# huggingface/parler-tts

Hardware: NVIDIA H100
Metric: audio codec tokens/sec (all codebooks) (higher is better)
Workload: dtype bf16

## Files before the change

### parler_tts_b200/csrc/step2.cu

```cuda
#include "attn_core.cuh"
#include "common.cuh"
#include "kernels.h"
#include "ln_stats.cuh"
#include "sample_core.cuh"
#include "ptx.cuh"
#include "step.h"
#include "step_common.cuh"
#include <type_traits>

namespace ptts {
namespace cl {

constexpr int C = 2;
constexpr int V = 8;
constexpr int THREADS = 256;
constexpr int ROWS = 32;
constexpr int HROWS = 8;
constexpr int ATT_SMEM = attn_decode_smem_per_warp<bf16>();
constexpr int PROF_STRIDE = 16;
constexpr int QMAX = 6;
constexpr int OFF_STATS = 256, OFF_PART = 512, OFF_RES = 2560, OFF_CVEC = 3584;
constexpr int HDR = 5632;
constexpr int WB_BYTES = 65536;
constexpr int R_OFF = HDR + 2 * WB_BYTES;
constexpr int R_BYTES = 92160;
constexpr int R_PASS0 = 65536;
constexpr int QKV_OFF = R_BYTES - 2048;
constexpr int SMEM_BYTES = R_OFF + R_BYTES;
static_assert(SMEM_BYTES + 1024 <= 227 * 1024, "cluster step kernel shared memory");
static_assert(ROWS * (1024 / 2 + 8) * 2 <= V * (256 + ROWS * 34 * 4) && 2 * V * (256 + ROWS * 34 * 4) <= R_BYTES, "fc1 plan");
static_assert(2 * V * C * (32 + 4 * 96 * 4) <= R_PASS0 && R_PASS0 + V * QMAX * 32 * 16 <= QKV_OFF, "QKV plan");
static_assert(5 * ATT_SMEM <= QKV_OFF && 3 * ATT_SMEM <= WB_BYTES && 16384 + 4 * 128 * 4 <= WB_BYTES, "attention plan");
static_assert(ROWS * (4096 / 4 + 8) * 2 + V * (256 + ROWS * 8 * 4) <= R_BYTES, "fc2 plan");

__device__ __forceinline__ void mbar_wait(uint64_t* bar, uint32_t parity, int what) {
  uint32_t ok, spins = 0;
  do {
    ok = mbar_try_wait_cluster(bar, parity);
    if (!ok && ++spins > (1u << 22)) { printf("ptts: cluster step mbarrier timeout (cta %d, barrier kind %d)\n", (int)blockIdx.x, what); __trap(); }
  } while (!ok);
}
__device__ __forceinline__ void bulk_s2peer(uint32_t dst_cluster_addr, const void* src_smem, uint32_t bytes, uint32_t bar_cluster_addr) {
  asm volatile("cp.async.bulk.shared::cluster.shared::cta.mbarrier::complete_tx::bytes [%0], [%1], %2, [%3];"
               ::"r"(dst_cluster_addr), "r"(smem_u32(src_smem)), "r"(bytes), "r"(bar_cluster_addr) : "memory");
}
__device__ __forceinline__ uint32_t mapa(uint32_t addr, uint32_t rank) { uint32_t r; asm volatile("mapa.shared::cluster.u32 %0, %1, %2;" : "=r"(r) : "r"(addr), "r"(rank)); return r; }
__device__ __forceinline__ uint32_t cluster_rank() { uint32_t r; asm volatile("mov.u32 %0, %%cluster_ctarank;" : "=r"(r)); return r; }
__device__ __forceinline__ void cluster_arrive() { asm volatile("barrier.cluster.arrive.release.aligned;" ::: "memory"); }
__device__ __forceinline__ void cluster_wait() { asm volatile("barrier.cluster.wait.acquire.aligned;" ::: "memory"); }
__device__ __forceinline__ void cluster_arrive_reuse() { asm volatile("barrier.cluster.arrive.relaxed.aligned;" ::: "memory"); }

__host__ __device__ __forceinline__ int kslice(int kt) { return (kt & 7) >> 2; }
__host__ __device__ __forceinline__ int klocal(int kt) { return ((kt >> 3) << 2) | (kt & 3); }
__host__ __device__ __forceinline__ int kglobal(int rank, int lk) { return ((lk >> 2) << 3) | (rank << 2) | (lk & 3); }

template <int QN, int MT, bool STATS, bool ACC = false>
__device__ __forceinline__ void mma_slice(float (&out)[2][6][4], RowStatFrag& rst, const bf16* xs, int apitch, const uint4* wb, int KT, int kt0,
                                          int kt_end, int lrow, int lcol) {
  float acc[MT][QN][4];
#pragma unroll
  for (int a = 0; a < MT; a++)
#pragma unroll
    for (int j = 0; j < QN; j++)
#pragma unroll
      for (int e = 0; e < 4; e++) acc[a][j][e] = ACC ? out[a][j][e] : 0.f;
  for (int kt = kt0; kt < kt_end; kt += 4) {
    uint32_t a[MT][2][4];
#pragma unroll
    for (int mt = 0; mt < MT; mt++)
#pragma unroll
      for (int j = 0; j < 2; j++) ldmatrix_x4(a[mt][j], xs + (size_t)(mt * 16 + lrow) * apitch + kt * 32 + j * 16 + lcol);
    if (STATS) {
#pragma unroll
      for (int mt = 0; mt < MT; mt++) { row_stat_mma(rst, mt, a[mt][0]); row_stat_mma(rst, mt, a[mt][1]); }
    }
#pragma unroll
    for (int j = 0; j < QN; j++) {
      const uint4 w = wb[((size_t)j * KT + kt) * 32];
#pragma unroll
      for (int mt = 0; mt < MT; mt++) {
        mma_bf16_16816(acc[mt][j], a[mt][0], w.x, w.y);
        mma_bf16_16816(acc[mt][j], a[mt][1], w.z, w.w);
      }
    }
  }
#pragma unroll
  for (int mt = 0; mt < MT; mt++)
#pragma unroll
    for (int j = 0; j < QN; j++)
#pragma unroll
      for (int e = 0; e < 4; e++) out[mt][j][e] = acc[mt][j][e];
}

enum { PH_QKV = 0, PH_O = 1, PH_QC = 2, PH_OC = 3, PH_FC1 = 4, PH_FC2 = 5 };
constexpr int JOBS_PER_LAYER = 9;
constexpr int QKV_JOBS = 4;

__device__ __forceinline__ bool weight_job(const StepParams& p, int j, int cta, int rank, const char*& src, uint32_t& bytes) {
  const int nl = JOBS_PER_LAYER * p.L;
  if (j < nl) {
    const int l = j / JOBS_PER_LAYER, jl = j - JOBS_PER_LAYER * l;
    const int ph = jl < QKV_JOBS ? 0 : jl - (QKV_JOBS - 1);
    const int64_t idx = (ph == PH_QKV || ph == PH_QC) ? (int64_t)(cta >> 3) * C + rank : (int64_t)cta;
    const int64_t sz = p.cp_slice[ph];
    bytes = (uint32_t)(ph == PH_QKV ? sz / QKV_JOBS : sz);
    src = p.blob + p.layer0 + p.layer_stride * l + p.cp[ph] + idx * sz + (ph == PH_QKV ? jl * (sz / QKV_JOBS) : 0);
    return true;
  }
  const int task = cta + (int)gridDim.x * (j - nl);
  const int ntasks = p.K * p.V / 32;
  if (task >= ntasks) return false;
  bytes = (uint32_t)(4 * p.H * 16);
  src = p.blob + p.heads + (int64_t)task * bytes;
  return true;
}

template <int ITEMS>
__global__ void __launch_bounds__(THREADS, 1) decode_step_cluster_kernel(const __grid_constant__ StepParams p) {
  extern __shared__ __align__(128) unsigned char smem[];
  Ctrl* ctrl = p.sa.ctrl;
  if (p.prof != nullptr && blockIdx.x == 0 && threadIdx.x == 0) p.prof[(size_t)(6 * p.L + 2) * PROF_STRIDE + 3] = clock64();
  if (ctrl->active == 0) return;
  int cur_len = ctrl->cur_len;
  const unsigned gen = (unsigned)ctrl->launch_gen;
  int pos = p.P + cur_len - 1;
  const int tid = threadIdx.x, warp = tid >> 5, lane = tid & 31;
  const int H = p.H, F = p.F, B = p.B;
  const int rank = (int)cluster_rank();
  const int cta = (int)blockIdx.x;
  const int cluster = cta >> 1;
  const int head = cluster >> 2, rblk = cluster & 3;
  const int Ks = H / C, KsF = F / 4;
  const int pitch = Ks + 8, pitchF = KsF + 8;
  const int qe = F / p.nh / 64;
  const int dgrp = warp & 1, e4 = warp >> 1;

  uint64_t* abar = reinterpret_cast<uint64_t*>(smem);
  uint64_t* wbar = abar + 1;
  uint64_t* xbar = abar + 3;
  uint64_t* attbars = reinterpret_cast<uint64_t*>(smem + 128);
  float* stats = reinterpret_cast<float*>(smem + OFF_STATS);
  float* part = reinterpret_cast<float*>(smem + OFF_PART);
  float* res_s = reinterpret_cast<float*>(smem + OFF_RES);
  float* cvec = reinterpret_cast<float*>(smem + OFF_CVEC);
  unsigned char* Rg = smem + R_OFF;
  uint32_t par_a = 0, par_w = 0, par_x = 0, att_parity = 0;

  if (tid == 0) {
    mbar_init<1>(abar); mbar_init<1>(&wbar[0]); mbar_init<1>(&wbar[1]); mbar_init<1>(xbar);
    asm volatile("fence.mbarrier_init.release.cluster;" ::: "memory");
  }
  attention_decode_init_warp(attbars + 2 * warp, lane);
  cluster_arrive(); cluster_wait();
  unsigned* const bar_ctr = p.bar + (gen & 1u);
  unsigned bar_target = 0u;
  if (cta == 0 && tid == 0) p.bar[(gen + 1u) & 1u] = 0u;

  const char* blob = p.blob;
  long long* const prof0 = (p.prof != nullptr && cta == 0) ? p.prof : nullptr;
  long long* prof = prof0;
  prof_mark(prof, 0);

  auto issue_weight_job = [&](int j) {
    const char* src; uint32_t bytes;
    if (!weight_job(p, j, cta, rank, src, bytes)) return;
    mbar_expect_tx(&wbar[j & 1], bytes);
    bulk_g2s_evict_first(smem + HDR + (j & 1) * WB_BYTES, src, bytes, &wbar[j & 1]);
  };
  __shared__ int s_next_active;
  const int n_steps = (p.do_sample_phase && p.n_steps > 1 && prof0 == nullptr) ? p.n_steps : 1;
  int unfinished_prev = 0;
#pragma unroll 1
  for (int it = 0; it < n_steps; it++) {
  pos = p.P + cur_len - 1;
  prof = prof0;
  cluster_arrive_reuse();
  if (tid == 0) { issue_weight_job(0); issue_weight_job(1); }

  bf16* const x_img = p.cl_x;
  bf16* const a_img = p.cl_attn;
  bf16* const h_img = p.cl_h;
  const int x_slice_elems = ROWS * pitch, h_slice_elems = ROWS * pitchF;
  auto h_offset = [&](int n) {
    const int lk = klocal(n >> 5), kq = KsF >> 5;
    return (size_t)(2 * kslice(n >> 5) + lk / kq) * h_slice_elems + (lk % kq) * 32 + (n & 31);
  };
  const int xo_slice = kslice(cta >> 2), xo_col = klocal(cta >> 2) * 32 + (cta & 3) * 8;

  {
    const int row = tid >> 3, f = tid & 7, n = cta * 8 + f;
    const float v = row < B ? embed_value(p, row, n, pos) : 0.f;
    res_s[row * 8 + f] = v;
    x_img[(size_t)xo_slice * x_slice_elems + row * pitch + xo_col + f] = __float2bfloat16_rn(v);
  }
  prof_mark(prof, 6);
  auto request_slice = [&](const bf16* img_slice, uint32_t bytes) {
    fence_proxy_async_smem();
    mbar_expect_tx(abar, bytes);
    bulk_g2s(Rg, img_slice, bytes, abar);
  };
  auto slice_of = [&](int sub, const bf16*& img, uint32_t& bytes) {
    if (sub == PH_QKV || sub == PH_QC) { img = x_img + (size_t)rank * x_slice_elems + (size_t)(HROWS * rblk) * pitch; bytes = (uint32_t)(HROWS * pitch * 2); }
    else if (sub == PH_O || sub == PH_OC) { img = a_img + (size_t)rank * x_slice_elems; bytes = (uint32_t)(x_slice_elems * 2); }
    else if (sub == PH_FC1) { img = x_img + (size_t)rank * x_slice_elems; bytes = (uint32_t)(x_slice_elems * 2); }
    else { img = h_img + (size_t)(2 * rank) * h_slice_elems; bytes = (uint32_t)(h_slice_elems * 2); }
  };
  {
    const bf16* nimg; uint32_t nbytes;
    slice_of(PH_QKV, nimg, nbytes);
    bar_target = grid_sync(bar_ctr, bar_target, -1, false, nullptr, [&]() { request_slice(nimg, nbytes); });
  }
  prof_mark(prof, 7);

  const int lrow = (lane & 7) + ((lane >> 3) & 1) * 8, lcol = (lane >> 4) * 8;
  const int g = lane >> 2, t4 = lane & 3;
  const int n_phases = 6 * p.L;

  const int att_row = HROWS * rblk + 4 * rank + (warp >> 1);
  const int att_slice = kslice(2 * head), att_col = klocal(2 * head) * 32;

#pragma unroll 1
  for (int ph = 0; ph < n_phases; ph++) {
    const int l = ph / 6, sub = ph - 6 * l;
    prof = prof0 ? prof0 + (size_t)(ph + 1) * PROF_STRIDE : nullptr;
    prof_mark(prof, 0);
    const char* lb = blob + p.layer0 + p.layer_stride * l;
    const bool rowpart = (sub == PH_QKV || sub == PH_QC);
    const bool has_ln = (sub == PH_QKV || sub == PH_QC || sub == PH_FC1);
    const int q = (sub == PH_QKV) ? 6 : (sub == PH_QC ? 2 : (sub == PH_FC1 ? qe : 1));
    const int Nc = 4 * q * 8;
    const int KT = (sub == PH_FC2 ? KsF : Ks) >> 5;
    const int apitch = (sub == PH_FC2) ? pitchF : pitch;
    const int act_bytes = (rowpart ? HROWS : ROWS) * apitch * 2;
    const int RS = (q == 1) ? 8 : 8 * q + 2;
    const int blk = rowpart ? 32 + 4 * 16 * q * 4 : 256 + ROWS * RS * 4;
    const int wsend = rowpart ? C * blk : blk;
    const int j0 = JOBS_PER_LAYER * l + (sub == 0 ? 0 : sub + QKV_JOBS - 1);

    float cv1 = 0.f, cv2 = 0.f;
    if (has_ln) {
      const float* c1; int ntot;
      if (sub == PH_QKV) { c1 = reinterpret_cast<const float*>(lb + p.c_qkv); ntot = p.qkv_rows; }
      else if (sub == PH_QC) { c1 = reinterpret_cast<const float*>(lb + p.c_qc); ntot = H; }
      else { c1 = reinterpret_cast<const float*>(lb + p.c_fc1); ntot = F; }
      const int nown = rowpart ? Nc : 8 * q;
      if (tid < nown) {
        int n;
        if (sub == PH_QKV) n = (tid >> 6) * (p.nh * HD) + head * HD + (tid & 63);
        else if (sub == PH_QC) n = head * HD + tid;
        else n = cta * 8 * q + tid;
        cv1 = c1[n];
        cv2 = c1[ntot + n];
      }
    }

    auto wait_job = [&](int j) {
      mbar_wait(&wbar[j & 1], (par_w >> (j & 1)) & 1u, 1);
      par_w ^= 1u << (j & 1);
    };
    auto ring = [&](int j) { return reinterpret_cast<const uint4*>(smem + HDR + (j & 1) * WB_BYTES) + lane; };
    wait_job(j0);
    if (sub == PH_QKV) wait_job(j0 + 1);
    mbar_wait(abar, par_a, 0);
    par_a ^= 1u;
    prof_mark(prof, 1);
    float acc[2][QMAX][4];
    float4* const pass0 = reinterpret_cast<float4*>(Rg + R_PASS0) + (size_t)warp * QMAX * 32 + lane;
    RowStatFrag rst;
    row_stat_zero(rst);
    {
      const bf16* xs = reinterpret_cast<const bf16*>(Rg);
      if (rowpart) {
        auto head_pass = [&](auto pass_tag) {
          constexpr int P = decltype(pass_tag)::value;
          const int u = 2 * P + dgrp;
          float t[2][QMAX][4];
          if (sub == PH_QKV) mma_slice<6, 1, P == 0>(t, rst, xs, apitch, ring(j0 + u), KT, e4, KT, lrow & 7, lcol);
          else mma_slice<2, 1, P == 0>(t, rst, xs, apitch, ring(j0) + (size_t)(2 * u) * KT * 32, KT, e4, KT, lrow & 7, lcol);
#pragma unroll
          for (int j = 0; j < QMAX; j++)
            if (j < q) {
              if (P == 0) pass0[j * 32] = make_float4(t[0][j][0], t[0][j][1], t[0][j][2], t[0][j][3]);
              else {
#pragma unroll
                for (int e = 0; e < 4; e++) acc[0][j][e] = t[0][j][e];
              }
            }
        };
        head_pass(std::integral_constant<int, 0>{});
        if (sub == PH_QKV) {
          prof_mark(prof, 8);
          __syncthreads();
          if (tid == 0) { issue_weight_job(j0 + 2); issue_weight_job(j0 + 3); }
          wait_job(j0 + 2);
          wait_job(j0 + 3);
          prof_mark(prof, 9);
        }
        head_pass(std::integral_constant<int, 1>{});
      } else if (sub == PH_FC2) {
        auto quarter = [&](auto qq_tag) {
          constexpr int QQ = decltype(qq_tag)::value;
          const uint4* wq = ring(j0) + (size_t)dgrp * 2 * KT * 32 + (size_t)QQ * KT * 32;
          mma_slice<1, 2, false, QQ == 1>(acc, rst, xs, apitch, wq, 2 * KT, (e4 - QQ * KT) & 3, KT, lrow, lcol);
        };
        quarter(std::integral_constant<int, 0>{});
        prof_mark(prof, 8);
        __syncthreads();
        if (tid == 0) request_slice(h_img + (size_t)(2 * rank + 1) * h_slice_elems, (uint32_t)(h_slice_elems * 2));
        mbar_wait(abar, par_a, 0);
        par_a ^= 1u;
        prof_mark(prof, 9);
        quarter(std::integral_constant<int, 1>{});
      } else {
        const uint4* wb = ring(j0) + (size_t)(dgrp * q) * KT * 32;
        if (sub == PH_FC1) {
          if (q == 4) mma_slice<4, 2, true>(acc, rst, xs, apitch, wb, KT, e4, KT, lrow, lcol);
          else if (q == 2) mma_slice<2, 2, true>(acc, rst, xs, apitch, wb, KT, e4, KT, lrow, lcol);
          else mma_slice<1, 2, true>(acc, rst, xs, apitch, wb, KT, e4, KT, lrow, lcol);
        } else mma_slice<1, 2, false>(acc, rst, xs, apitch, wb, KT, e4, KT, lrow, lcol);
      }
    }
    prof_mark(prof, 2);
    if (has_ln && tid < (rowpart ? Nc : 8 * q)) { cvec[tid] = cv1; cvec[256 + tid] = cv2; }
    __syncthreads();
    prof_mark(prof, 12);
    cluster_wait();
    prof_mark(prof, 13);

    const int nslots = rowpart ? V * C : V;
    unsigned char* send = Rg;
    const int send_end = V * wsend;
    unsigned char* recv = Rg + (((send_end > act_bytes ? send_end : act_bytes) + 127) & ~127);
    if (tid == 0) mbar_expect_tx(xbar, (uint32_t)(nslots * blk));
    {
      unsigned char* mine = send + (size_t)warp * wsend;
      if (!rowpart) {
        float* bp = reinterpret_cast<float*>(mine + 256);
#pragma unroll
        for (int mt = 0; mt < 2; mt++)
#pragma unroll
          for (int j = 0; j < QMAX; j++) {
            if (j < q) {
              float* base = bp + (size_t)(mt * 16 + g) * RS + j * 8 + 2 * t4;
              *reinterpret_cast<float2*>(base) = make_float2(acc[mt][j][0], acc[mt][j][1]);
              *reinterpret_cast<float2*>(base + 8 * RS) = make_float2(acc[mt][j][2], acc[mt][j][3]);
            }
          }
        if (has_ln) {
          float* st = reinterpret_cast<float*>(mine);
#pragma unroll
          for (int mt = 0; mt < 2; mt++) {
            const int r0 = mt * 16 + g;
            if (t4 == 0) { st[2 * r0] = rst.s1[mt][0]; st[2 * (r0 + 8)] = rst.s1[mt][2]; }
            if (t4 == (g >> 1)) {
              st[2 * r0 + 1] = (g & 1) ? rst.sq[mt][0][1] : rst.sq[mt][0][0];
              st[2 * (r0 + 8) + 1] = (g & 1) ? rst.sq[mt][1][3] : rst.sq[mt][1][2];
            }
          }
        }
      } else {
        const int qc = 16 * q;
        unsigned char* blk_d = send + ((size_t)(g >> 2) * V + warp) * blk;
        float* bp = reinterpret_cast<float*>(blk_d + 32) + (g & 3) * qc + 2 * t4;
#pragma unroll
        for (int P = 0; P < 2; P++)
#pragma unroll
          for (int j = 0; j < QMAX; j++)
            if (j < q) *reinterpret_cast<float2*>(bp + P * 8 * q + j * 8) = P == 0 ? make_float2(pass0[j * 32].x, pass0[j * 32].y)
                                                                                   : make_float2(acc[0][j][0], acc[0][j][1]);
        float* st = reinterpret_cast<float*>(blk_d) + (g & 3) * 2;
        if (t4 == 0) st[0] = rst.s1[0][0];
        if (t4 == (g >> 1)) st[1] = (g & 1) ? rst.sq[0][0][1] : rst.sq[0][0][0];
      }
      __syncwarp();
      prof_mark(prof, 14);
      if (!rowpart) {
        if (lane == 0) {
          fence_proxy_async_smem();
          bulk_s2peer(mapa(smem_u32(recv + (size_t)(4 * rank + e4) * blk), (uint32_t)dgrp), mine, (uint32_t)blk, mapa(smem_u32(xbar), (uint32_t)dgrp));
        }
      } else {
        __syncthreads();
        if (warp < C && lane == 0) {
          fence_proxy_async_smem();
          bulk_s2peer(mapa(smem_u32(recv + (size_t)(8 * rank) * blk), (uint32_t)warp), send + (size_t)warp * V * blk, (uint32_t)(V * blk), mapa(smem_u32(xbar), (uint32_t)warp));
        }
      }
    }
    if (warp == 1 && lane == 0 && !rowpart && sub != PH_OC) issue_weight_job(j0 + 2);
    if (warp == 1 && lane == 0 && sub == PH_QKV) issue_weight_job(j0 + QKV_JOBS);
    prof_mark(prof, 15);
    mbar_wait(xbar, par_x, 2);
    par_x ^= 1u;
    prof_mark(prof, 3);

    if (!rowpart) {
      const int row = tid >> 3, f0 = tid & 7;
      float ln_mean = 0.f, ln_rstd = 0.f;
      if (has_ln) {
        float S1 = 0.f, S2 = 0.f;
#pragma unroll
        for (int v = 0; v < V; v++) { const float2 x = *reinterpret_cast<const float2*>(recv + (size_t)v * blk + row * 8); S1 += x.x; S2 += x.y; }
        ln_mean = S1 / (float)H;
        ln_rstd = rsqrtf(fmaxf(S2 / (float)H - ln_mean * ln_mean, 0.f) + p.eps);
      }
      if (row < B && sub == PH_FC1 && q == 4) {
        const int f = 4 * f0;
        float v[4] = {0.f, 0.f, 0.f, 0.f};
#pragma unroll
        for (int sv = 0; sv < V; sv++) {
          const float* bp = reinterpret_cast<const float*>(recv + (size_t)sv * blk + 256) + row * RS + f;
          const float2 a = *reinterpret_cast<const float2*>(bp), b2 = *reinterpret_cast<const float2*>(bp + 2);
          v[0] += a.x; v[1] += a.y; v[2] += b2.x; v[3] += b2.y;
        }
#pragma unroll
        for (int e = 0; e < 4; e++) v[e] = apply_act(DT<bf16>::rnd(ln_rstd * (v[e] - ln_mean * cvec[f + e]) + cvec[256 + f + e]), p.act);
        uint2 pk;
        pk.x = att_pack(v[0], v[1]); pk.y = att_pack(v[2], v[3]);
        *reinterpret_cast<uint2*>(h_img + h_offset(cta * 32 + f) + row * pitchF) = pk;
      } else if (row < B) {
        for (int i = 0; i < q; i++) {
          const int f = f0 + 8 * i;
          float v = 0.f;
#pragma unroll
          for (int sv = 0; sv < V; sv++) v += reinterpret_cast<const float*>(recv + (size_t)sv * blk + 256)[row * RS + f];
          if (sub == PH_FC1) {
            v = ln_rstd * (v - ln_mean * cvec[f]) + cvec[256 + f];
            v = apply_act(DT<bf16>::rnd(v), p.act);
            h_img[h_offset(cta * 8 * q + f) + row * pitchF] = __float2bfloat16_rn(v);
          } else {
            v = DT<bf16>::rnd(res_s[row * 8 + f] + DT<bf16>::rnd(v));
            res_s[row * 8 + f] = v;
            x_img[(size_t)xo_slice * x_slice_elems + row * pitch + xo_col + f] = __float2bfloat16_rn(v);
          }
        }
      }
    } else {
      bf16* qkv_s = reinterpret_cast<bf16*>(Rg + QKV_OFF);
      auto gather = [&](auto jw_tag) {
        constexpr int JW = decltype(jw_tag)::value, NC = 4 * JW, QCW = 2 * JW;
        for (int idx = tid; idx < 4 * NC; idx += THREADS) {
          const int r4 = idx / NC, col = idx - r4 * NC;
          const int u = col / JW, cw = (u >> 1) * JW + (col - u * JW);
          float S1 = 0.f, S2 = 0.f;
#pragma unroll
          for (int e = 0; e < V; e++) {
            const float2 x = *reinterpret_cast<const float2*>(recv + (size_t)(8 * (e >> 2) + 2 * (e & 3)) * blk + r4 * 8);
            S1 += x.x; S2 += x.y;
          }
          const float ln_mean = S1 / (float)H;
          const float ln_rstd = rsqrtf(fmaxf(S2 / (float)H - ln_mean * ln_mean, 0.f) + p.eps);
          float v = 0.f;
#pragma unroll
          for (int e = 0; e < V; e++)
            v += reinterpret_cast<const float*>(recv + (size_t)(8 * (e >> 2) + 2 * (e & 3) + (u & 1)) * blk + 32)[r4 * QCW + cw];
          v = ln_rstd * (v - ln_mean * cvec[col]) + cvec[256 + col];
          qkv_s[idx] = __float2bfloat16_rn(v);
        }
      };
      if (sub == PH_QKV) gather(std::integral_constant<int, 48>{}); else gather(std::integral_constant<int, 16>{});
      static_assert(HD == 64, "QKV: 2 x 2 units of 6 n-tiles (q|k|v of a head), q_cross: 2 x 2 units of 2 n-tiles");
    }
    prof_mark(prof, 4);
    __syncthreads();
    cluster_arrive_reuse();
    if (rowpart) {
      cluster_wait();
      cluster_arrive();
    }

    if (rowpart) {
      if (att_row < B) {
        AttnArgs att = decode_attn_args(p, l, pos, sub == PH_QC);
        const bf16* qkv_s = reinterpret_cast<const bf16*>(Rg + QKV_OFF);
        const int row_base = HROWS * rblk + 4 * rank;
        const bf16* qbase = qkv_s - (size_t)row_base * Nc - (size_t)head * HD;
        att.q = qbase; att.ldq = Nc;
        att.ldo = pitch;
        att.out = a_img + (size_t)att_slice * x_slice_elems + att_col - (size_t)head * HD;
        if (sub == PH_QKV) { att.knew = qbase; att.vnew = qbase; att.ldkv = Nc; att.k_col0 = HD; att.v_col0 = 2 * HD; }
        unsigned char* wb0 = smem + HDR;
        unsigned char* held = wb0 + ((sub == PH_QKV ? j0 + 1 : j0) & 1) * WB_BYTES;
        unsigned char* other = wb0 + ((sub == PH_QKV ? j0 : j0 + 1) & 1) * WB_BYTES;
        unsigned char* region = warp < 5 ? Rg + (size_t)warp * ATT_SMEM : held + (size_t)(warp - 5) * ATT_SMEM;
        float* xr = reinterpret_cast<float*>(other + 16384) + (warp >> 1) * 128;
        attention_decode_item_warp<bf16>(att, att_row, head, pos, region, attbars + 2 * warp, lane, att_parity, warp & 1, 2, xr, (warp >> 1) + 1);
      }
      prof_mark(prof, 5);
    }
    prof_mark(prof, 6);
    if (p.prof != nullptr && l == p.L / 2 && tid == 0) {
      unsigned long long ns;
      asm volatile("mov.u64 %0, %%globaltimer;" : "=l"(ns));
      p.prof[(size_t)(n_phases + 4) * PROF_STRIDE + sub * (int)gridDim.x + cta] = (long long)ns;
    }

    const bool last = (ph + 1 == n_phases);
    const bf16* nimg; uint32_t nbytes;
    if (last) { nimg = x_img; nbytes = (uint32_t)(C * x_slice_elems * 2); }
    else slice_of((sub + 1) % 6, nimg, nbytes);
    const int held_job = sub == PH_QKV ? j0 + QKV_JOBS + 1 : (sub == PH_QC || sub == PH_OC) ? j0 + 2 : -1;
    bar_target = grid_sync(bar_ctr, bar_target, ph, false, nullptr, [&]() {
      request_slice(nimg, nbytes);
      if (held_job >= 0) issue_weight_job(held_job);
    });
    prof_mark(prof, 7);
  }
  cluster_wait();

  prof = prof0 ? prof0 + (size_t)(n_phases + 1) * PROF_STRIDE : nullptr;
  prof_mark(prof, 0);
  {
    const int ntasks = p.K * p.V / 32;
    const float* c1 = reinterpret_cast<const float*>(blob + p.c_heads);
    const float* c2 = c1 + p.K * p.V;
    mbar_wait(abar, par_a, 3);
    par_a ^= 1u;
    const bf16* xs = reinterpret_cast<const bf16*>(Rg);
    const int KTH = H >> 5;
    auto ktile = [&](int kt) { return xs + (size_t)kslice(kt) * x_slice_elems + klocal(kt) * 32; };
    {
      RowStatFrag rst;
      row_stat_zero(rst);
      for (int kt = warp; kt < KTH; kt += 8) {
        const bf16* sl = ktile(kt);
#pragma unroll
        for (int mt = 0; mt < 2; mt++)
#pragma unroll
          for (int j = 0; j < 2; j++) {
            uint32_t a[4];
            ldmatrix_x4(a, sl + (size_t)(mt * 16 + lrow) * pitch + j * 16 + lcol);
            row_stat_mma(rst, mt, a);
          }
      }
      row_stat_store(rst, part, warp, lane);
      __syncthreads();
      row_stat_finalize(part, H, ROWS, p.eps, stats);
      __syncthreads();
    }
    prof_mark(prof, 1);
    constexpr int HRS = 40;
    int job = JOBS_PER_LAYER * p.L;
    for (int task = cta; task < ntasks; task += (int)gridDim.x, job++) {
      mbar_wait(&wbar[job & 1], (par_w >> (job & 1)) & 1u, 4);
      par_w ^= 1u << (job & 1);
      float acc[2][4][4];
#pragma unroll
      for (int a = 0; a < 2; a++)
#pragma unroll
        for (int j = 0; j < 4; j++)
#pragma unroll
          for (int e = 0; e < 4; e++) acc[a][j][e] = 0.f;
      unsigned char* wbuf = smem + HDR + (job & 1) * WB_BYTES;
      const uint4* wb = reinterpret_cast<const uint4*>(wbuf) + lane;
      for (int kt = warp; kt < KTH; kt += 8) {
        const bf16* sl = ktile(kt);
        uint32_t a[2][2][4];
#pragma unroll
        for (int mt = 0; mt < 2; mt++)
#pragma unroll
          for (int j = 0; j < 2; j++) ldmatrix_x4(a[mt][j], sl + (size_t)(mt * 16 + lrow) * pitch + j * 16 + lcol);
#pragma unroll
        for (int j = 0; j < 4; j++) {
          const uint4 w = wb[((size_t)j * KTH + kt) * 32];
#pragma unroll
          for (int mt = 0; mt < 2; mt++) {
            mma_bf16_16816(acc[mt][j], a[mt][0], w.x, w.y);
            mma_bf16_16816(acc[mt][j], a[mt][1], w.z, w.w);
          }
        }
      }
      __syncthreads();
      float* red = reinterpret_cast<float*>(wbuf);
#pragma unroll
      for (int mt = 0; mt < 2; mt++)
#pragma unroll
        for (int j = 0; j < 4; j++) {
          float* base = red + ((size_t)warp * 32 + mt * 16 + g) * HRS + j * 8 + 2 * t4;
          *reinterpret_cast<float2*>(base) = make_float2(acc[mt][j][0], acc[mt][j][1]);
          *reinterpret_cast<float2*>(base + 8 * HRS) = make_float2(acc[mt][j][2], acc[mt][j][3]);
        }
      __syncthreads();
      {
        const int er = tid >> 3, ec = tid & 7;
        if (er < B) {
          const float mean = stats[2 * er], rstd = stats[2 * er + 1];
#pragma unroll
          for (int j = 0; j < 4; j++) {
            const int cidx = j * 8 + ec, n = task * 32 + cidx;
            float v = 0.f;
#pragma unroll
            for (int w = 0; w < 8; w++) v += red[((size_t)w * 32 + er) * HRS + cidx];
            p.logits[(size_t)er * p.K * p.V + n] = DT<bf16>::rnd(rstd * (v - mean * c1[n]) + c2[n]);
          }
        }
      }
      __syncthreads();
      if (tid == 32) {
        fence_proxy_async_smem();
        issue_weight_job(job + 2);
      }
    }
  }
  prof_mark(prof, 6);
  bar_target = grid_sync(bar_ctr, bar_target, n_phases, true);
  prof = prof0 ? prof0 + (size_t)(n_phases + 2) * PROF_STRIDE : nullptr;
  prof_mark(prof, 0);
  if (p.do_sample_phase) {
    const ptts_gen_params gp = *p.sa.gen;
    const int BK = B * p.K;
    sample_phase<ITEMS>(p.sa, gp, BK, cur_len);
    prof_mark(prof, 1);
    bar_target = grid_sync(bar_ctr, bar_target, n_phases + 1, true, nullptr, [&]() {
      const int tot = *reinterpret_cast<volatile int*>(&ctrl->n_unfinished);
      s_next_active = (tot - unfinished_prev > 0) ? 1 : 0;
      unfinished_prev = tot;
    });
    prof_mark(prof, 2);
  }
  bool go_on = false;
  if (p.do_sample_phase) {
    const int act = s_next_active;
    if (cta == 0 && tid == 0) {
      ctrl->cur_len = cur_len + 1;
      ctrl->active = act;
      ctrl->steps_run += 1;
    }
    go_on = act != 0;
    cur_len += 1;
  }
  if (!go_on) break;
  }
  if (cta == 0 && tid == 0) {
    if (p.do_sample_phase) ctrl->n_unfinished = 0;
    ctrl->launch_gen = (int)(gen + 1u);
  }
}

__global__ void cluster_pack_kernel(const uint4* __restrict__ src, uint4* __restrict__ dst, int ph, int nh, int ntc, int kts, int KT_src) {
  const int64_t tile = blockIdx.x;
  const int ktl = (int)(tile % kts);
  const int j = (int)((tile / kts) % ntc);
  const int slice = (int)(tile / ((int64_t)kts * ntc));
  const int rank = slice & 1, owner = slice >> 1;
  int n_tile;
  if (ph == PH_QKV) n_tile = (j >> 3) * (nh * 8) + owner * 8 + (j & 7);
  else n_tile = owner * ntc + j;
  const int kt = kglobal(rank, ktl);
  dst[tile * 32 + threadIdx.x] = src[((int64_t)n_tile * KT_src + kt) * 32 + threadIdx.x];
}

}

int cluster_pack_layer(const char* layer_src, char* layer_dst, const int64_t* mat_off, const int64_t* cp_off, int nh, int H, int F, cudaStream_t st) {
  const int ks = H / cl::C / 32, ksf = F / cl::C / 32;
  const int ntc[6] = {24, 2, 8, 2, F / (4 * nh) / 8, 2};
  const int owners[6] = {nh, 4 * nh, nh, 4 * nh, 4 * nh, 4 * nh};
  for (int ph = 0; ph < 6; ph++) {
    const int kts = (ph == 5) ? ksf : ks;
    const int KT_src = (ph == 5) ? F / 32 : H / 32;
    const int64_t tiles = (int64_t)owners[ph] * cl::C * ntc[ph] * kts;
    cl::cluster_pack_kernel<<<(unsigned)tiles, 32, 0, st>>>(reinterpret_cast<const uint4*>(layer_src + mat_off[ph]),
                                                            reinterpret_cast<uint4*>(layer_dst + cp_off[ph]), ph, nh, ntc[ph], kts, KT_src);
  }
  PTTS_LAUNCH_CHECK();
  return PTTS_OK;
}

static const void* cluster_kernel_fn(const StepParams& p) {
  if (p.sample_items <= 1) return (const void*)cl::decode_step_cluster_kernel<1>;
  if (p.sample_items <= 5) return (const void*)cl::decode_step_cluster_kernel<5>;
  return (const void*)cl::decode_step_cluster_kernel<9>;
}

static void cluster_launch_config(const StepParams& p, cudaLaunchConfig_t& cfg, cudaLaunchAttribute* at, cudaStream_t st) {
  cfg = cudaLaunchConfig_t{};
  cfg.gridDim = dim3((unsigned)(4 * p.nh * cl::C));
  cfg.blockDim = dim3(cl::THREADS);
  cfg.dynamicSmemBytes = cl::SMEM_BYTES;
  cfg.stream = st;
  at[0].id = cudaLaunchAttributeClusterDimension;
  at[0].val.clusterDim.x = cl::C; at[0].val.clusterDim.y = 1; at[0].val.clusterDim.z = 1;
  at[1].id = cudaLaunchAttributeCooperative;
  at[1].val.cooperative = 1;
  cfg.attrs = at;
  cfg.numAttrs = 2;
}

bool cluster_step_available(const StepParams& p) {
  const void* fn = cluster_kernel_fn(p);
  static bool told = false;
  auto why = [&](const char* what, cudaError_t e, int n) {
    if (!told) fprintf(stderr, "ptts_b200: cluster step kernel not used (%s: %s, %d co-resident clusters of %d, need %d); the one-CTA-per-SM step kernel runs instead\n",
                       what, cudaGetErrorString(e), n, cl::C, 4 * p.nh);
    told = true;
    cudaGetLastError();
    return false;
  };
  cudaError_t e = cudaFuncSetAttribute(fn, cudaFuncAttributeMaxDynamicSharedMemorySize, cl::SMEM_BYTES);
  if (e != cudaSuccess) return why("shared memory attribute", e, 0);
  cudaLaunchConfig_t cfg; cudaLaunchAttribute at[2];
  cluster_launch_config(p, cfg, at, nullptr);
  cfg.numAttrs = 1;
  int n = 0;
  e = cudaOccupancyMaxActiveClusters(&n, fn, &cfg);
  if (e != cudaSuccess) return why("cluster occupancy query", e, n);
  if (n < 4 * p.nh) return why("too few co-resident clusters", cudaSuccess, n);
  return true;
}

int launch_decode_step_cluster(const StepParams& p, cudaStream_t st) {
  const void* fn = cluster_kernel_fn(p);
  cudaLaunchConfig_t cfg; cudaLaunchAttribute at[2];
  cluster_launch_config(p, cfg, at, st);
  void* args[] = {(void*)&p};
  PTTS_CHECK_CUDA(cudaLaunchKernelExC(&cfg, fn, args));
  return PTTS_OK;
}

}
```

Baseline: 228,500.

## Exchange partial GEMM results via per-thread st.async into peer CTA shared memory

Replaces the staged exchange of partial matmul results and layernorm stats with direct st.async stores from registers into the peer CTA's receive buffer (or local stores for the own rank). Previously these were written to a local send buffer, then moved with a bulk cp.async after syncthreads and syncwarp. The change drops the send staging area, the pass-0 spill buffer, and an extra cluster wait/arrive round in row-partitioned phases. The mbarrier expected-tx count is now computed analytically, so it must match the number of bytes actually stored remotely. That adds many small remote stores and some ordering risk around cluster_wait placement.

```diff
diff --git a/parler_tts_b200/csrc/step2.cu b/parler_tts_b200/csrc/step2.cu
--- a/parler_tts_b200/csrc/step2.cu
+++ b/parler_tts_b200/csrc/step2.cu
@@ -24,12 +24,11 @@
 constexpr int WB_BYTES = 65536;
 constexpr int R_OFF = HDR + 2 * WB_BYTES;
 constexpr int R_BYTES = 92160;
-constexpr int R_PASS0 = 65536;
 constexpr int QKV_OFF = R_BYTES - 2048;
 constexpr int SMEM_BYTES = R_OFF + R_BYTES;
 static_assert(SMEM_BYTES + 1024 <= 227 * 1024, "cluster step kernel shared memory");
-static_assert(ROWS * (1024 / 2 + 8) * 2 <= V * (256 + ROWS * 34 * 4) && 2 * V * (256 + ROWS * 34 * 4) <= R_BYTES, "fc1 plan");
-static_assert(2 * V * C * (32 + 4 * 96 * 4) <= R_PASS0 && R_PASS0 + V * QMAX * 32 * 16 <= QKV_OFF, "QKV plan");
+static_assert(ROWS * (1024 / 2 + 8) * 2 + V * (256 + ROWS * 34 * 4) <= R_BYTES, "fc1 plan");
+static_assert(HROWS * (1024 / 2 + 8) * 2 + V * C * (32 + 4 * 96 * 4) <= QKV_OFF, "QKV plan");
 static_assert(5 * ATT_SMEM <= QKV_OFF && 3 * ATT_SMEM <= WB_BYTES && 16384 + 4 * 128 * 4 <= WB_BYTES, "attention plan");
 static_assert(ROWS * (4096 / 4 + 8) * 2 + V * (256 + ROWS * 8 * 4) <= R_BYTES, "fc2 plan");
 
@@ -40,9 +39,13 @@
     if (!ok && ++spins > (1u << 22)) { printf("ptts: cluster step mbarrier timeout (cta %d, barrier kind %d)\n", (int)blockIdx.x, what); __trap(); }
   } while (!ok);
 }
-__device__ __forceinline__ void bulk_s2peer(uint32_t dst_cluster_addr, const void* src_smem, uint32_t bytes, uint32_t bar_cluster_addr) {
-  asm volatile("cp.async.bulk.shared::cluster.shared::cta.mbarrier::complete_tx::bytes [%0], [%1], %2, [%3];"
-               ::"r"(dst_cluster_addr), "r"(smem_u32(src_smem)), "r"(bytes), "r"(bar_cluster_addr) : "memory");
+__device__ __forceinline__ void st_async(uint32_t dst_cluster_addr, float v, uint32_t bar_cluster_addr) {
+  asm volatile("st.async.shared::cluster.mbarrier::complete_tx::bytes.b32 [%0], %1, [%2];"
+               ::"r"(dst_cluster_addr), "r"(__float_as_uint(v)), "r"(bar_cluster_addr) : "memory");
+}
+__device__ __forceinline__ void st_async(uint32_t dst_cluster_addr, float2 v, uint32_t bar_cluster_addr) {
+  asm volatile("st.async.shared::cluster.mbarrier::complete_tx::bytes.v2.f32 [%0], {%1, %2}, [%3];"
+               ::"r"(dst_cluster_addr), "f"(v.x), "f"(v.y), "r"(bar_cluster_addr) : "memory");
 }
 __device__ __forceinline__ uint32_t mapa(uint32_t addr, uint32_t rank) { uint32_t r; asm volatile("mapa.shared::cluster.u32 %0, %1, %2;" : "=r"(r) : "r"(addr), "r"(rank)); return r; }
 __device__ __forceinline__ uint32_t cluster_rank() { uint32_t r; asm volatile("mov.u32 %0, %%cluster_ctarank;" : "=r"(r)); return r; }
@@ -126,7 +129,7 @@
   int pos = p.P + cur_len - 1;
   const int tid = threadIdx.x, warp = tid >> 5, lane = tid & 31;
   const int H = p.H, F = p.F, B = p.B;
-  const int rank = (int)cluster_rank();
+  const int rank = (int)cluster_rank(), peer = rank ^ 1;
   const int cta = (int)blockIdx.x;
   const int cluster = cta >> 1;
   const int head = cluster >> 2, rblk = cluster & 3;
@@ -144,6 +147,7 @@
   float* res_s = reinterpret_cast<float*>(smem + OFF_RES);
   float* cvec = reinterpret_cast<float*>(smem + OFF_CVEC);
   unsigned char* Rg = smem + R_OFF;
+  const uint32_t peer_xbar = mapa(smem_u32(xbar), (uint32_t)peer);
   uint32_t par_a = 0, par_w = 0, par_x = 0, att_parity = 0;
 
   if (tid == 0) {
@@ -234,8 +238,15 @@
     const int act_bytes = (rowpart ? HROWS : ROWS) * apitch * 2;
     const int RS = (q == 1) ? 8 : 8 * q + 2;
     const int blk = rowpart ? 32 + 4 * 16 * q * 4 : 256 + ROWS * RS * 4;
-    const int wsend = rowpart ? C * blk : blk;
+    unsigned char* const recv = Rg + ((act_bytes + 127) & ~127);
+    const uint32_t peer_recv = mapa(smem_u32(recv), (uint32_t)peer);
+    const uint32_t xbytes = 4u * (rowpart ? V * 4 * 16 * q + V / 2 * 4 * 2 : V / C * (ROWS * 8 * q + (has_ln ? ROWS * 2 : 0)));
+    auto put = [&](int d, uint32_t off, auto v) {
+      if (d == rank) *reinterpret_cast<decltype(v)*>(recv + off) = v;
+      else st_async(peer_recv + off, v, peer_xbar);
+    };
     const int j0 = JOBS_PER_LAYER * l + (sub == 0 ? 0 : sub + QKV_JOBS - 1);
+    if (tid == 0) mbar_expect_tx(xbar, xbytes);
 
     float cv1 = 0.f, cv2 = 0.f;
     if (has_ln) {
@@ -265,7 +276,6 @@
     par_a ^= 1u;
     prof_mark(prof, 1);
     float acc[2][QMAX][4];
-    float4* const pass0 = reinterpret_cast<float4*>(Rg + R_PASS0) + (size_t)warp * QMAX * 32 + lane;
     RowStatFrag rst;
     row_stat_zero(rst);
     {
@@ -277,15 +287,19 @@
           float t[2][QMAX][4];
           if (sub == PH_QKV) mma_slice<6, 1, P == 0>(t, rst, xs, apitch, ring(j0 + u), KT, e4, KT, lrow & 7, lcol);
           else mma_slice<2, 1, P == 0>(t, rst, xs, apitch, ring(j0) + (size_t)(2 * u) * KT * 32, KT, e4, KT, lrow & 7, lcol);
+          const int d = g >> 2;
+          const uint32_t slot = (uint32_t)((8 * rank + warp) * blk);
+          if (P == 0) {
+            cluster_wait();
+            if (dgrp == 0) {
+              const uint32_t so = slot + 8 * (g & 3);
+              if (t4 == 0) put(d, so, rst.s1[0][0]);
+              if (t4 == (g >> 1)) put(d, so + 4, (g & 1) ? rst.sq[0][0][1] : rst.sq[0][0][0]);
+            }
+          }
 #pragma unroll
           for (int j = 0; j < QMAX; j++)
-            if (j < q) {
-              if (P == 0) pass0[j * 32] = make_float4(t[0][j][0], t[0][j][1], t[0][j][2], t[0][j][3]);
-              else {
-#pragma unroll
-                for (int e = 0; e < 4; e++) acc[0][j][e] = t[0][j][e];
-              }
-            }
+            if (j < q) put(d, slot + 32 + 4 * ((g & 3) * 16 * q + P * 8 * q + j * 8 + 2 * t4), make_float2(t[0][j][0], t[0][j][1]));
         };
         head_pass(std::integral_constant<int, 0>{});
         if (sub == PH_QKV) {
@@ -321,72 +335,36 @@
       }
     }
     prof_mark(prof, 2);
+    prof_mark(prof, 12);
+    if (!rowpart) cluster_wait();
+    prof_mark(prof, 13);
+    if (!rowpart) {
+      const uint32_t slot = (uint32_t)((4 * rank + e4) * blk);
+#pragma unroll
+      for (int mt = 0; mt < 2; mt++)
+#pragma unroll
+        for (int j = 0; j < QMAX; j++) {
+          if (j < q) {
+            const uint32_t o = slot + 256 + 4 * ((mt * 16 + g) * RS + j * 8 + 2 * t4);
+            put(dgrp, o, make_float2(acc[mt][j][0], acc[mt][j][1]));
+            put(dgrp, o + 4 * 8 * RS, make_float2(acc[mt][j][2], acc[mt][j][3]));
+          }
+        }
+      if (has_ln) {
+#pragma unroll
+        for (int mt = 0; mt < 2; mt++) {
+          const uint32_t s0 = slot + 8 * (mt * 16 + g), s8 = s0 + 8 * 8;
+          if (t4 == 0) { put(dgrp, s0, rst.s1[mt][0]); put(dgrp, s8, rst.s1[mt][2]); }
+          if (t4 == (g >> 1)) {
+            put(dgrp, s0 + 4, (g & 1) ? rst.sq[mt][0][1] : rst.sq[mt][0][0]);
+            put(dgrp, s8 + 4, (g & 1) ? rst.sq[mt][1][3] : rst.sq[mt][1][2]);
+          }
+        }
+      }
+    }
+    prof_mark(prof, 14);
     if (has_ln && tid < (rowpart ? Nc : 8 * q)) { cvec[tid] = cv1; cvec[256 + tid] = cv2; }
     __syncthreads();
-    prof_mark(prof, 12);
-    cluster_wait();
-    prof_mark(prof, 13);
-
-    const int nslots = rowpart ? V * C : V;
-    unsigned char* send = Rg;
-    const int send_end = V * wsend;
-    unsigned char* recv = Rg + (((send_end > act_bytes ? send_end : act_bytes) + 127) & ~127);
-    if (tid == 0) mbar_expect_tx(xbar, (uint32_t)(nslots * blk));
-    {
-      unsigned char* mine = send + (size_t)warp * wsend;
-      if (!rowpart) {
-        float* bp = reinterpret_cast<float*>(mine + 256);
-#pragma unroll
-        for (int mt = 0; mt < 2; mt++)
-#pragma unroll
-          for (int j = 0; j < QMAX; j++) {
-            if (j < q) {
-              float* base = bp + (size_t)(mt * 16 + g) * RS + j * 8 + 2 * t4;
-              *reinterpret_cast<float2*>(base) = make_float2(acc[mt][j][0], acc[mt][j][1]);
-              *reinterpret_cast<float2*>(base + 8 * RS) = make_float2(acc[mt][j][2], acc[mt][j][3]);
-            }
-          }
-        if (has_ln) {
-          float* st = reinterpret_cast<float*>(mine);
-#pragma unroll
-          for (int mt = 0; mt < 2; mt++) {
-            const int r0 = mt * 16 + g;
-            if (t4 == 0) { st[2 * r0] = rst.s1[mt][0]; st[2 * (r0 + 8)] = rst.s1[mt][2]; }
-            if (t4 == (g >> 1)) {
-              st[2 * r0 + 1] = (g & 1) ? rst.sq[mt][0][1] : rst.sq[mt][0][0];
-              st[2 * (r0 + 8) + 1] = (g & 1) ? rst.sq[mt][1][3] : rst.sq[mt][1][2];
-            }
-          }
-        }
-      } else {
-        const int qc = 16 * q;
-        unsigned char* blk_d = send + ((size_t)(g >> 2) * V + warp) * blk;
-        float* bp = reinterpret_cast<float*>(blk_d + 32) + (g & 3) * qc + 2 * t4;
-#pragma unroll
-        for (int P = 0; P < 2; P++)
-#pragma unroll
-          for (int j = 0; j < QMAX; j++)
-            if (j < q) *reinterpret_cast<float2*>(bp + P * 8 * q + j * 8) = P == 0 ? make_float2(pass0[j * 32].x, pass0[j * 32].y)
-                                                                                   : make_float2(acc[0][j][0], acc[0][j][1]);
-        float* st = reinterpret_cast<float*>(blk_d) + (g & 3) * 2;
-        if (t4 == 0) st[0] = rst.s1[0][0];
-        if (t4 == (g >> 1)) st[1] = (g & 1) ? rst.sq[0][0][1] : rst.sq[0][0][0];
-      }
-      __syncwarp();
-      prof_mark(prof, 14);
-      if (!rowpart) {
-        if (lane == 0) {
-          fence_proxy_async_smem();
-          bulk_s2peer(mapa(smem_u32(recv + (size_t)(4 * rank + e4) * blk), (uint32_t)dgrp), mine, (uint32_t)blk, mapa(smem_u32(xbar), (uint32_t)dgrp));
-        }
-      } else {
-        __syncthreads();
-        if (warp < C && lane == 0) {
-          fence_proxy_async_smem();
-          bulk_s2peer(mapa(smem_u32(recv + (size_t)(8 * rank) * blk), (uint32_t)warp), send + (size_t)warp * V * blk, (uint32_t)(V * blk), mapa(smem_u32(xbar), (uint32_t)warp));
-        }
-      }
-    }
     if (warp == 1 && lane == 0 && !rowpart && sub != PH_OC) issue_weight_job(j0 + 2);
     if (warp == 1 && lane == 0 && sub == PH_QKV) issue_weight_job(j0 + QKV_JOBS);
     prof_mark(prof, 15);
@@ -464,10 +442,6 @@
     prof_mark(prof, 4);
     __syncthreads();
     cluster_arrive_reuse();
-    if (rowpart) {
-      cluster_wait();
-      cluster_arrive();
-    }
 
     if (rowpart) {
       if (att_row < B) {
```

Result: faster. 239,600 (median of 6 runs) (+4.9%).
